# dusanerdeljan/stereo-depth

Hardware: AMD Instinct MI355X
Metric: disparity maps/sec (stereo pairs/sec) at 1242x375 D=128 (higher is better)
Workload: dtype f32

## Files before the change

stereo-depth_amd/csrc/k_match_fast.h:

```cpp
#pragma once
#include "smx_common.h"

namespace smx {

constexpr int FA_HALO = 11;
constexpr int FA_VALID = 64 - 2 * FA_HALO;
#ifndef SMX_FA_WAVES
#define SMX_FA_WAVES 4
#endif
constexpr int FA_WAVES = SMX_FA_WAVES;
#ifndef SMX_FA_DS_WAVES
#define SMX_FA_DS_WAVES 8
#endif
constexpr int FA_DS_WAVES = SMX_FA_DS_WAVES;
#ifndef SMX_FA_TH
#define SMX_FA_TH 24
#endif
constexpr int FA_TH = SMX_FA_TH;
#ifndef SMX_FA_TH_SMALL
#define SMX_FA_TH_SMALL 8
#endif
constexpr int FA_TH_SMALL = SMX_FA_TH_SMALL;
constexpr int FA_TH_SMALL_TALL = 12;
constexpr int FA_TH_SMALL_MID = 10;
#ifndef SMX_FA_PF
#define SMX_FA_PF 2
#endif
constexpr int FA_PF = SMX_FA_PF;
#ifndef SMX_FA_SB_PERIOD
#define SMX_FA_SB_PERIOD 2
#endif
#ifndef SMX_FA_OCC
#define SMX_FA_OCC 3
#endif
#ifndef SMX_FA_DS_OCC
#define SMX_FA_DS_OCC 4
#endif
constexpr int FA_WGCOLS = FA_VALID * FA_WAVES + 2 * FA_HALO;
#ifndef SMX_FA_WIDE_FROM
#define SMX_FA_WIDE_FROM (256 - FA_WGCOLS + 1)
#endif
constexpr int FA_WIDE_FROM = SMX_FA_WIDE_FROM;
constexpr int FA_MID_PITCH = 288;
#ifdef SMX_FA_NO_MID_PITCH
constexpr int FA_MID_UPTO = 0;
#else
constexpr int FA_MID_UPTO = FA_MID_PITCH - FA_WGCOLS + 1;
#endif
constexpr int FA_PL = (FA_VALID * FA_WAVES + 2 * FA_HALO + 7) & ~7;
constexpr int FA_BITWORDS = 64;
__host__ __device__ inline int fast_bitwords(int Dd) {
    return Dd > FA_BITWORDS * 32 ? 2 : ((Dd + 1) & ~1);
}
#define SMX_FOR_EACH_NEEDED(tbl, lo, hi, all_needed, lane, dd, rows, BODY)                                      \
    for (int g_ = (lo); g_ < (hi); g_ += 64) {                                                                  \
        const int idx_ = g_ + (lane);                                                                           \
        unsigned word_ = 0u;                                                                                    \
        if (idx_ < (hi)) word_ = (all_needed) ? ~0u : (tbl)[idx_];                                              \
        unsigned long long m_ = __ballot(word_ != 0u);                                                          \
        while (m_ != 0ull) {                                                                                    \
            const int k_ = __builtin_ctzll(m_);                                                                 \
            m_ &= m_ - 1ull;                                                                                    \
            const int dd = g_ + k_;                                                                             \
            const unsigned rows = (unsigned)__builtin_amdgcn_readlane((int)word_, k_);                          \
            BODY                                                                                                \
        }                                                                                                       \
    }

constexpr int FA_DENSE_MAX_TH = 27;
constexpr int FA_XROW = 64 + 12;
#ifndef SMX_FA_XCH_ROWS
#define SMX_FA_XCH_ROWS 2
#endif
constexpr int FA_XCH_ROWS = SMX_FA_XCH_ROWS;
constexpr int FA_XCH_FLOATS = 2 * FA_XCH_ROWS * FA_XROW;

__host__ __device__ constexpr int fast_merge_rows(int th) { return th > 8 ? (th + 1) / 2 : th; }

template <int PR> inline size_t fast_lds_bytes(int th, int Dd, bool dsplit = false) {
    const size_t nw = dsplit ? FA_DS_WAVES : FA_WAVES;
    return (size_t)(th + 22) * (FA_PL + PR) * sizeof(unsigned short) + nw * fast_bitwords(Dd) * sizeof(unsigned) +
           nw * FA_XCH_FLOATS * sizeof(float) + (dsplit ? nw * fast_merge_rows(th) * 64 * 2 * sizeof(float) : 0);
}

__device__ __forceinline__ float dpp_shr1(float v) {
    return __int_as_float(__builtin_amdgcn_update_dpp(0, __float_as_int(v), 0x138, 0xf, 0xf, true));
}
__device__ __forceinline__ float dpp_shl1(float v) {
    return __int_as_float(__builtin_amdgcn_update_dpp(0, __float_as_int(v), 0x130, 0xf, 0xf, true));
}
__device__ __forceinline__ unsigned dppu_sum3(unsigned v) {
    unsigned t = (unsigned)__builtin_amdgcn_update_dpp(0, (int)v, 0x138, 0xf, 0xf, true) + v;
    asm("" : "+v"(t));
    return t + (unsigned)__builtin_amdgcn_update_dpp(0, (int)v, 0x130, 0xf, 0xf, true);
}

__device__ __forceinline__ void store_u32off(float *base_uniform, unsigned off_elems, float v) {
    *(float *)((char *)base_uniform + (size_t)(off_elems * 4u)) = v;
}

__device__ __forceinline__ void atomic_or_u32off(unsigned *base_uniform, unsigned off_words, unsigned bits) {
    atomicOr((unsigned *)((char *)base_uniform + (size_t)(off_words * 4u)), bits);
}

template <int NK, int NW, bool ROUND = false>
__device__ __forceinline__ void fast_stage(unsigned short *tile, int pitch, const float *img, int h, int w,
                                           int row0, int col0, int rows, int cols, float unit, int wv, int lane) {
    int cidx[NK];
    {
        int c = wrapi(col0 + lane, w);
        const int cstep = 64 % w;
#pragma unroll
        for (int k = 0; k < NK; ++k) {
            cidx[k] = c;
            c += cstep;
            c = c >= w ? c - w : c;
        }
    }
    int ra = wrapi(row0 + wv, h);
    const int rstep = (2 * NW) % h, rhalf = NW % h;
    for (int r = wv; r < rows; r += 2 * NW) {
        const int r2 = r + NW;
        int rb = ra + rhalf;
        rb = rb >= h ? rb - h : rb;
        const float *src = img + (size_t)ra * w;
        const float *src2 = img + (size_t)(r2 < rows ? rb : ra) * w;
        float v[NK], v2[NK];
#pragma unroll
        for (int k = 0; k < NK; ++k) {
            const bool in = lane + 64 * k < cols;
            v[k] = in ? src[cidx[k]] : 0.f;
            v2[k] = in ? src2[cidx[k]] : 0.f;
        }
        unsigned short *dst = tile + r * pitch, *dst2 = tile + r2 * pitch;
#pragma unroll
        for (int k = 0; k < NK; ++k) {
            if (lane + 64 * k < cols) {
                dst[lane + 64 * k] = (unsigned short)(ROUND ? unit * v[k] + 0.5f : unit * v[k]);
                if (r2 < rows) dst2[lane + 64 * k] = (unsigned short)(ROUND ? unit * v2[k] + 0.5f : unit * v2[k]);
            }
        }
        ra += rstep;
        ra = ra >= h ? ra - h : ra;
    }
}

struct FastLane {
    const unsigned short *lptr, *rptr;
    float *xch;
    unsigned c255;
    float inv;
    bool store_ok;
    int rows_ok;
    int colidx;
    size_t row0;
    size_t plane;
    unsigned *cand;
    unsigned cand_off_a, cand_off_b;
    unsigned long long cand_mask_a, cand_mask_b;
    unsigned cand_rstride;
    int x0;
};

typedef float f32x2 __attribute__((ext_vector_type(2)));
typedef __attribute__((address_space(3))) f32x2 fa_lds_f32x2;

__device__ __forceinline__ void argb_update(int kbyte, int &word, float m, float best, int dsel) {
    if (kbyte == 0)
        asm volatile("v_cmp_gt_f32 vcc, %1, %2\n\tv_cndmask_b32_sdwa %0, %0, %3, vcc dst_sel:BYTE_0 dst_unused:UNUSED_PRESERVE src0_sel:BYTE_0 src1_sel:BYTE_0"
                     : "+v"(word) : "v"(m), "v"(best), "v"(dsel) : "vcc");
    else if (kbyte == 1)
        asm volatile("v_cmp_gt_f32 vcc, %1, %2\n\tv_cndmask_b32_sdwa %0, %0, %3, vcc dst_sel:BYTE_1 dst_unused:UNUSED_PRESERVE src0_sel:BYTE_1 src1_sel:BYTE_0"
                     : "+v"(word) : "v"(m), "v"(best), "v"(dsel) : "vcc");
    else if (kbyte == 2)
        asm volatile("v_cmp_gt_f32 vcc, %1, %2\n\tv_cndmask_b32_sdwa %0, %0, %3, vcc dst_sel:BYTE_2 dst_unused:UNUSED_PRESERVE src0_sel:BYTE_2 src1_sel:BYTE_0"
                     : "+v"(word) : "v"(m), "v"(best), "v"(dsel) : "vcc");
    else
        asm volatile("v_cmp_gt_f32 vcc, %1, %2\n\tv_cndmask_b32_sdwa %0, %0, %3, vcc dst_sel:BYTE_3 dst_unused:UNUSED_PRESERVE src0_sel:BYTE_3 src1_sel:BYTE_0"
                     : "+v"(word) : "v"(m), "v"(best), "v"(dsel) : "vcc");
}

template <int TH, int PR, bool P1ONLY, int PK16, int MODE = 0, bool ARGB = false, bool DENSE = false>
__device__ __forceinline__ void fast_pass_pair(const MatchParams &p, const FastLane &ln, int d,
                                               bool valid_b, float (&best)[TH], int (&arg)[TH],
                                               const unsigned short *rptr_b_in = nullptr, int db = 0,
                                               const unsigned *argpk = nullptr, int am_a = 0, int ap_a = 0,
                                               int am_b = 0, int ap_b = 0, const unsigned *vpk = nullptr,
                                               unsigned *hits = nullptr, unsigned rowmask = ~0u,
                                               float *dmb = nullptr, float *dma = nullptr, float *dcp = nullptr,
                                               float *dfirst = nullptr) {
    constexpr int NQ = TH + 20;
    f32x2 s1 = {0.f, 0.f}, s2 = {0.f, 0.f};
    unsigned k1 = 0u, k2 = 0u;
    const unsigned c255pk = ln.c255 * 0x10001u;
    f32x2 r3[NQ], r9[NQ], r21[NQ];
    unsigned lv[TH + 22], rva[TH + 22], rvb[TH + 22];
    f32x2 vs = {0.f, 0.f}, cs = {0.f, 0.f}, hs = {0.f, 0.f};
    f32x2 t_m3 = {0.f, 0.f}, t_p3 = {0.f, 0.f}, u_m6 = {0.f, 0.f}, u_p6 = {0.f, 0.f};
    const int lane_ = threadIdx.x & 63;
#ifdef SMX_FA_ARGMAX2
    int dva = d, dvb = d + 1;
    if (ARGB && MODE == 0) asm volatile("" : "+v"(dva), "+v"(dvb));
#endif
    const unsigned short *rptr_b = (MODE == 0 || MODE == 3) ? ln.rptr - (valid_b ? 1 : 0) : rptr_b_in;
    (void)db;
#pragma unroll
    for (int rr_ = 0; rr_ < TH + 22 + FA_PF; ++rr_) {
        if (rr_ < TH + 22) {
            lv[rr_] = ln.lptr[rr_ * FA_PL];
            rva[rr_] = ln.rptr[rr_ * PR];
            rvb[rr_] = rptr_b[rr_ * PR];
        }
        if (rr_ >= FA_PF) {
            const int r = rr_ - FA_PF;
            f32x2 s0 = {0.f, 0.f};
            unsigned k0 = 0u;
            if (PK16) {
                const unsigned sa = __builtin_amdgcn_sad_u16(lv[r], rva[r], 0u);
                const unsigned sb = __builtin_amdgcn_sad_u16(lv[r], rvb[r], 0u);
                k0 = c255pk - ((sb << 16) | sa);
            } else {
                s0.x = (float)(ln.c255 - __builtin_amdgcn_sad_u16(lv[r], rva[r], 0u));
                s0.y = (float)(ln.c255 - __builtin_amdgcn_sad_u16(lv[r], rvb[r], 0u));
            }
            if (r >= 2) {
                const int q = r - 2;
                f32x2 x3;
                if (PK16 == 2) {
                    const unsigned v3 = (k2 + k1) + k0;
                    const unsigned cv = dppu_sum3(v3);
                    const unsigned y3 = dppu_sum3(cv);
                    x3.x = (float)(y3 & 0xffffu);
                    x3.y = (float)(y3 >> 16);
                } else if (PK16 == 1) {
                    const unsigned v3 = (k2 + k1) + k0;
                    const unsigned cvp = dppu_sum3(v3);
                    f32x2 cv;
                    cv.x = (float)(cvp & 0xffffu);
                    cv.y = (float)(cvp >> 16);
                    x3.x = (dpp_shr1(cv.x) + cv.x) + dpp_shl1(cv.x);
                    x3.y = (dpp_shr1(cv.y) + cv.y) + dpp_shl1(cv.y);
                } else {
                    const f32x2 v3 = (s2 + s1) + s0;
                    f32x2 cv;
                    cv.x = (dpp_shr1(v3.x) + v3.x) + dpp_shl1(v3.x);
                    cv.y = (dpp_shr1(v3.y) + v3.y) + dpp_shl1(v3.y);
                    x3.x = (dpp_shr1(cv.x) + cv.x) + dpp_shl1(cv.x);
                    x3.y = (dpp_shr1(cv.y) + cv.y) + dpp_shl1(cv.y);
                }
                r3[q] = x3;
                if (q >= 12) r9[q - 6] = (t_m3 + r3[q - 6]) + t_p3;
                if (q >= 18) r21[q - 9] = (u_m6 + u_p6) + r3[q - 9];
#ifdef SMX_EXP_NOXCH
                if (q >= 11 && q + 1 < NQ) { t_m3 = r3[q - 5]; t_p3 = r3[q - 4]; }
                if (q >= 17 && q + 1 < NQ) { u_m6 = r9[q - 8]; u_p6 = r9[q - 7]; }
#else
                if (q >= 11 && q + 1 < NQ) {
                    f32x2 *x3b = (f32x2 *)ln.xch + lane_;
                    x3b[6] = r3[q - 5];
                    __builtin_amdgcn_wave_barrier();
                    {
                        const volatile fa_lds_f32x2 *xr = (const volatile fa_lds_f32x2 *)x3b;
                        t_m3 = xr[3]; t_p3 = xr[9];
                    }
                }
                if (q >= 17 && q + 1 < NQ) {
                    f32x2 *x9b = (f32x2 *)(ln.xch + (FA_XCH_ROWS > 1 ? 2 * FA_XROW : 0)) + lane_;
                    x9b[6] = r9[q - 8];
                    __builtin_amdgcn_wave_barrier();
                    {
                        const volatile fa_lds_f32x2 *xr = (const volatile fa_lds_f32x2 *)x9b;
                        u_m6 = xr[0]; u_p6 = xr[12];
                    }
                }
#endif
                vs += r3[q];
                if (q >= 21) vs -= r3[q - 21];
                if (q >= 12) cs += r9[q - 6];
                if (q >= 21) cs -= r9[q - 15];
                if (q >= 18) hs += r21[q - 9];
                if (q >= 21) hs -= r21[q - 12];
                if (q >= 20) {
                    const int o = q - 20;
                    const f32x2 agg = (hs * vs) * cs;
                    if ((MODE == 1 || MODE == 2) && !((rowmask >> o) & 1u)) {
                    } else if (MODE == 2) {
                        unsigned upk_w = argpk[o >> 1], vpk_w = vpk[o >> 1];
                        asm volatile("" : "+v"(upk_w), "+v"(vpk_w));
                        const unsigned U = (upk_w >> (16 * (o & 1))) & 0xffffu;
                        const unsigned V = (vpk_w >> (16 * (o & 1))) & 0xffffu;
                        int ci = ln.colidx;
                        asm volatile("" : "+v"(ci));
                        const unsigned off = (unsigned)(o * p.w + ci);
                        float *cp = p.costs + ln.row0;
                        auto put = [&](unsigned dl1, unsigned o2, float v) {
                            const size_t pl = dl1 == 1u ? 0 : (dl1 == 2u ? 1 : 2);
                            cp[pl * ln.plane + o2] = v * ln.inv;
                        };
                        const unsigned a1 = (unsigned)(d + 1) - U, a2 = V + 1u - (unsigned)d, a3 = (unsigned)(am_a + 1) - U;
                        const unsigned b1 = (unsigned)(db + 1) - U, b2 = V + 1u - (unsigned)db;
                        if (a1 < 3u) put(a1, off, agg.x);
                        if (a2 < 3u) put(a2, off + 1u, agg.x);
                        if (a3 < 3u) put(a3, off, agg.x);
                        if (b1 < 3u) put(b1, off, agg.y);
                        if (b2 < 3u) put(b2, off + 1u, agg.y);
                    } else if (MODE == 4) {
                        best[o] = __builtin_fmaxf(__builtin_fmaxf(best[o], agg.x), agg.y);
                    } else if (MODE == 3) {
                        const bool okp = ln.store_ok && o < ln.rows_ok;
                        const unsigned long long ma = __ballot(okp && agg.x >= best[o]);
                        const unsigned long long mb = __ballot(okp && agg.y >= best[o]);
                        const unsigned tr = (unsigned)(((ln.x0 + o) >> 4) - (ln.x0 >> 4));
                        const unsigned h4 = ((ma & ln.cand_mask_a) != 0ull ? 1u : 0u) | ((ma & ln.cand_mask_b) != 0ull ? 2u : 0u) |
                                            ((mb & ln.cand_mask_a) != 0ull ? 4u : 0u) | ((mb & ln.cand_mask_b) != 0ull ? 8u : 0u);
                        *hits |= h4 << (4u * tr);
                    } else if (MODE == 1) {
                        const int a = (int)((argpk[o >> 1] >> (16 * (o & 1))) & 0xffffu);
                        int ci = ln.colidx;
                        asm volatile("" : "+v"(ci));
                        const unsigned off = (unsigned)(o * p.w + ci);
                        const bool xa = a == am_a, xb = a == ap_a;
                        if (xa || a == am_b) store_u32off(p.costs + ln.row0 + ln.plane, off, (xa ? agg.x : agg.y) * ln.inv);
                        if (xb || a == ap_b) store_u32off(p.costs + ln.row0 + 2 * ln.plane, off, (xb ? agg.x : agg.y) * ln.inv);
                    } else {
                        if constexpr (DENSE) {
                            const float after_d = valid_b ? agg.y : __builtin_nanf("");
                            dma[o] = (dma[o] != dma[o]) ? agg.x : dma[o];
                            const bool ca = (agg.x > best[o]) | (d == 0);
                            const float b1 = __builtin_fmaxf(best[o], agg.x);
                            dmb[o] = ca ? dcp[o] : dmb[o];
                            dma[o] = ca ? after_d : dma[o];
                            const bool cb = agg.y > b1;
                            dmb[o] = cb ? agg.x : dmb[o];
                            dma[o] = cb ? __builtin_nanf("") : dma[o];
                            dcp[o] = agg.y;
                            if (dfirst) dfirst[o] = agg.x;
                        }
#if !defined(SMX_FA_ARGMAX2)
                        const float m = __builtin_fmaxf(__builtin_fmaxf(best[o], agg.x), agg.y);
                        const int dsel = (agg.x == m) ? d : d + 1;
#ifndef SMX_EXP_NOARG
                        if (ARGB) {
                            argb_update(o & 3, arg[o >> 2], m, best[o], dsel);
                        } else {
                            const bool changed = m > best[o];
                            arg[o] = changed ? dsel : arg[o];
                        }
#else
                        (void)dsel;
#endif
                        best[o] = m;
#else
                        if (ARGB) {
                            argb_update(o & 3, arg[o >> 2], agg.x, best[o], dva);
                            best[o] = __builtin_fmaxf(best[o], agg.x);
                            argb_update(o & 3, arg[o >> 2], agg.y, best[o], dvb);
                            best[o] = __builtin_fmaxf(best[o], agg.y);
                        } else {
                            const float m = __builtin_fmaxf(__builtin_fmaxf(best[o], agg.x), agg.y);
                            const int dsel = (agg.x == m) ? d : d + 1;
                            arg[o] = m > best[o] ? dsel : arg[o];
                            best[o] = m;
                        }
#endif
                    }
                }
            }
            s2 = s1;
            s1 = s0;
            k2 = k1;
            k1 = k0;
        }
        if ((rr_ % SMX_FA_SB_PERIOD) == SMX_FA_SB_PERIOD - 1)
            __builtin_amdgcn_sched_barrier(0);
    }
}

constexpr int FA_STAT_WG_STRIDE_DS = 16;
template <bool DSPLIT>
__device__ __forceinline__ void fast_stats_report(const MatchParams &p, int b, int wg_lin, int wv, int marches, bool window) {
    if (!p.fast_stats || b % p.fast_stride != 0) return;
    if (DSPLIT && wg_lin % FA_STAT_WG_STRIDE_DS != 0) return;
    const bool win = window && (!DSPLIT || wv == 0);
    const unsigned long long v = ((unsigned long long)(unsigned)marches << 24) | (win ? 1ull : 0ull);
    if (v != 0ull) (void)__hip_atomic_fetch_add(p.fast_stats, v, __ATOMIC_RELAXED, __HIP_MEMORY_SCOPE_AGENT);
}

template <int TU, int NH, int PR, int PK16, class StageRight>
__device__ __forceinline__ void fast_stacked_tail(const MatchParams &p, const BlockIdx3 &blk, const FastLane &ln, const float (&best)[TU * NH],
                                                  const int (&argb)[TU * NH], const unsigned short *Rt, unsigned *bits, int wcol, int x0,
                                                  bool active, StageRight &&stage_right) {
    constexpr int ND = PR - FA_WGCOLS + 1;
    const int lane = threadIdx.x & 63, wv = threadIdx.x >> 6;
    const int h = p.h, w = p.w, Dd = p.Dd, BW = fast_bitwords(Dd);
    const bool all_needed = Dd > FA_BITWORDS * 32;
    unsigned *wbits = bits + wv * BW;
#pragma unroll
    for (int hh = 0; hh < NH; ++hh) {
        float bh[TU];
        int ah[TU];
#pragma unroll
        for (int o = 0; o < TU; ++o) {
            bh[o] = best[hh * TU + o];
            ah[o] = (argb[(hh * TU + o) >> 2] >> (8 * ((hh * TU + o) & 3))) & 0xff;
        }
        FastLane lh = ln;
        lh.lptr = ln.lptr + hh * TU * FA_PL;
        lh.row0 = ln.row0 + (size_t)(hh * TU) * w;
        lh.rows_ok = max(0, min(TU, h - x0 - hh * TU));
        const unsigned short *Rh = Rt + hh * TU * PR;
        unsigned dup_left = 0u;
#ifndef SMX_FA_NO_DEDUP
        if (!all_needed) {
#pragma unroll
            for (int o = 0; o < TU; ++o) {
                const int la = __builtin_amdgcn_update_dpp(-1, ah[o], 0x138, 0xf, 0xf, false);
                dup_left |= (la == ah[o] ? 1u : 0u) << o;
            }
            const int left_ok = __builtin_amdgcn_update_dpp(0, lh.store_ok ? 1 : 0, 0x138, 0xf, 0xf, false);
            if (!left_ok) dup_left = 0u;
        }
#endif
        if (lh.store_ok) {
#pragma unroll
            for (int o = 0; o < TU; ++o) {
                if (o < lh.rows_ok) {
                    const unsigned off = (unsigned)(o * w + lh.colidx);
                    store_u32off(p.wta + lh.row0, off, (float)ah[o] + (float)p.dmin);
                    const bool nv = !(bh[o] > SMX_FLT_MIN);
                    store_u32off(p.costs + lh.row0, off, nv ? 0.0f : bh[o] * lh.inv);
                    if (!all_needed && !((dup_left >> o) & 1u)) {
                        const int dn = (ah[o] + 1 == Dd) ? 0 : ah[o] + 1;
                        const int dp = (ah[o] == 0) ? Dd - 1 : ah[o] - 1;
                        atomicOr(&wbits[dn], 1u << o);
                        atomicOr(&wbits[dp], 1u << o);
                    }
                }
            }
        }
        int marches2 = 0;
        unsigned argpk[(TU + 1) / 2];
#pragma unroll
        for (int o = 0; o < (TU + 1) / 2; ++o) argpk[o] = 0u;
#pragma unroll
        for (int o = 0; o < TU; ++o)
            argpk[o >> 1] |= ((lh.store_ok && o < lh.rows_ok) ? (unsigned)ah[o] : 0xffffu) << (16 * (o & 1));
        for (int d0 = 0; d0 < Dd; d0 += ND) {
            const int nd = min(ND, Dd - d0);
            if (Dd > ND) stage_right(d0, nd);
            else __syncthreads();
            if (active) {
                auto march = [&](int dda, int ddb, unsigned rows) {
                    const int da = d0 + dda, db = d0 + ddb;
                    ++marches2;
                    lh.rptr = Rh + wcol + lane + (nd - 1 - dda);
                    fast_pass_pair<TU, PR, false, PK16, 1>(p, lh, da, false, bh, ah, Rh + wcol + lane + (nd - 1 - ddb), db, argpk,
                                                           da == 0 ? Dd - 1 : da - 1, da + 1 == Dd ? 0 : da + 1,
                                                           db == 0 ? Dd - 1 : db - 1, db + 1 == Dd ? 0 : db + 1, nullptr, nullptr, rows);
                };
                int pend = -1;
                unsigned pend_rows = 0u;
                SMX_FOR_EACH_NEEDED(wbits + d0, 0, nd, all_needed, lane, dd, rows, {
                    if (pend < 0) { pend = dd; pend_rows = rows; }
                    else { march(pend, dd, pend_rows | rows); pend = -1; }
                })
                if (pend >= 0) march(pend, pend, pend_rows);
            }
        }
        if (lane == 0) fast_stats_report<false>(p, blk.z, (int)(blk.x + gridDim.x * blk.y), wv, marches2, active && lh.rows_ok > 0);
        if (hh + 1 < NH)
            for (int e = lane; e < BW; e += 64) wbits[e] = 0u;
    }
}

template <int TH, int PR, bool P1ONLY, bool DSPLIT, int PK16, bool ARGB = false, bool DENSE = false>
__device__ __forceinline__ void match_fast_body(const MatchParams &p, const BlockIdx3 &blk) {
    static_assert(!DENSE || !P1ONLY, "the dense form is a pass 1 with neighbours: min_disparity = 0");
    static_assert(!DENSE || !DSPLIT || !ARGB, "latency shape: one register per winner");
    constexpr int NW = DSPLIT ? FA_DS_WAVES : FA_WAVES;
    constexpr int WGCOLS = DSPLIT ? 64 : FA_WGCOLS;
    constexpr int ND = PR - WGCOLS + 1;
    constexpr int NH = TH > 32 ? 2 : 1;
    constexpr int TU = TH / NH;
    static_assert(NH == 1 || (TH == 2 * TU && TU <= 32 && ARGB && !DSPLIT && !DENSE && !P1ONLY),
                  "stacked bands: two unit bands, byte-packed winners, throughput shape, sparse form");
    const int b = blk.z;

    extern __shared__ __attribute__((aligned(16))) unsigned short fsmem[];
    unsigned short *Lt = fsmem;
    unsigned short *Rt = fsmem + (TH + 22) * FA_PL;
    unsigned *bits = (unsigned *)(Rt + (TH + 22) * PR);
    const int BW = fast_bitwords(p.Dd);

    const int tid = threadIdx.x;
    const int lane = tid & 63;
    const int wv = tid >> 6;
    const int h = p.h, w = p.w, Dd = p.Dd;
    const int cwg0 = blk.x * (DSPLIT ? 1 : FA_WAVES) * FA_VALID;
    const int cw0 = cwg0 + (DSPLIT ? 0 : wv * FA_VALID);
    const int wcol = DSPLIT ? 0 : wv * FA_VALID;
    const bool active = cw0 < w;
    const int x0 = blk.y * TH;
    const int col = cw0 - FA_HALO + lane;
    const float *Lp = p.Ld + (size_t)b * h * w;
    const float *Rp = p.Rd + (size_t)b * h * w;
    const float unit = p.unit;

    FastLane ln;
    ln.xch = (float *)(bits + NW * BW) + wv * FA_XCH_FLOATS;
    ln.c255 = (unsigned)(255.0f * unit);
    ln.inv = 1.0f / (unit * unit * unit);
    ln.store_ok = active && lane >= FA_HALO && lane < FA_HALO + FA_VALID && col < w;
    ln.rows_ok = min(TH, h - x0);
    ln.plane = (size_t)p.B * h * w;
    ln.row0 = ((size_t)b * h + x0) * w;
    ln.colidx = ln.store_ok ? col : 0;
    ln.lptr = Lt + wcol + lane;

    float best[TH];
    int arg[TH];
#pragma unroll
    for (int o = 0; o < TH; ++o) { best[o] = SMX_FLT_MIN; arg[o] = 0; }
    float dmb[DENSE ? TH : 1], dma[DENSE ? TH : 1], dcp[DENSE ? TH : 1];
    float dfirst[DENSE && DSPLIT ? TH : 1];
#pragma unroll
    for (int o = 0; o < (DENSE ? TH : 1); ++o) { dmb[o] = 0.f; dma[o] = 0.f; dcp[o] = 0.f; }
#pragma unroll
    for (int o = 0; o < (DENSE && DSPLIT ? TH : 1); ++o) dfirst[o] = 0.f;

    fast_stage<(WGCOLS + 63) / 64, NW>(Lt, FA_PL, Lp, h, w, x0 - FA_HALO, cwg0 - FA_HALO, TH + 22, WGCOLS, unit, wv, lane);
    for (int e = tid; e < NW * BW; e += 64 * NW) bits[e] = 0u;

    auto stage_right = [&](int d0, int nd) {
        __syncthreads();
        const int cbase = cwg0 - FA_HALO - (p.dmin + d0 + nd - 1);
        fast_stage<(PR + 63) / 64, NW>(Rt, PR, Rp, h, w, x0 - FA_HALO, cbase, TH + 22, WGCOLS + nd - 1, unit, wv, lane);
        __syncthreads();
    };

    for (int d0 = 0; d0 < Dd; d0 += ND) {
        const int nd = min(ND, Dd - d0);
        stage_right(d0, nd);
        if (active) {
            const int q4 = ((nd + 2 * NW - 1) / (2 * NW)) * 2;
            const int dd_lo = DSPLIT ? min(nd, wv * q4) : 0;
            const int dd_hi = DSPLIT ? min(nd, dd_lo + q4) : nd;
            for (int dd = dd_lo; dd < dd_hi; dd += 2) {
                ln.rptr = Rt + wcol + lane + (nd - 1 - dd);
                if constexpr (DENSE)
                    fast_pass_pair<TH, PR, P1ONLY, PK16, 0, ARGB, true>(p, ln, d0 + dd, dd + 1 < dd_hi, best, arg, nullptr, 0, nullptr,
                                                                         0, 0, 0, 0, nullptr, nullptr, ~0u, dmb, dma, dcp,
                                                                         DSPLIT && dd == dd_lo ? dfirst : nullptr);
                else
                    fast_pass_pair<TH, PR, P1ONLY, PK16, 0, ARGB>(p, ln, d0 + dd, dd + 1 < dd_hi, best, arg);
            }
        }
    }
    if constexpr (NH > 1) {
        fast_stacked_tail<TU, NH, PR, PK16>(p, blk, ln, best, arg, Rt, bits, wcol, x0, active, stage_right);
        return;
    }
    if (ARGB) {
        int packed[(TH + 3) / 4];
#pragma unroll
        for (int o = 0; o < (TH + 3) / 4; ++o) packed[o] = arg[o];
#pragma unroll
        for (int o = 0; o < TH; ++o) arg[o] = (packed[o >> 2] >> (8 * (o & 3))) & 0xff;
    }
    float *mrg = (float *)(bits + NW * BW) + NW * FA_XCH_FLOATS;
    if constexpr (DSPLIT && DENSE) {
        constexpr int MR = fast_merge_rows(TH), R2 = (NW * MR * 2) / (NW * 6);
        static_assert(R2 >= 1 && R2 <= NW, "merge buffer: at least one row of six values per wave");
        const int q4 = ((Dd + 2 * NW - 1) / (2 * NW)) * 2;
        const int nk = (Dd + q4 - 1) / q4;
#pragma unroll 1
        for (int o0 = 0; o0 < TH; o0 += R2) {
            __syncthreads();
#pragma unroll
            for (int o = 0; o < TH; ++o) {
                if (o >= o0 && o < o0 + R2) {
                    float *q = mrg + ((size_t)(wv * R2 + (o - o0)) * 64 + lane) * 6;
                    q[0] = best[o]; q[1] = __int_as_float(arg[o]); q[2] = dmb[o]; q[3] = dma[o]; q[4] = dfirst[o]; q[5] = dcp[o];
                }
            }
            __syncthreads();
            const int j = wv;
            if (j < R2 && o0 + j < ln.rows_ok && ln.store_ok) {
                auto M = [&](int k, int f) { return mrg[((size_t)(k * R2 + j) * 64 + lane) * 6 + f]; };
                float bb = SMX_FLT_MIN;
                int aa = 0, kw = 0;
                for (int k = 0; k < nk; ++k) {
                    const float bk = M(k, 0);
                    const bool g = bk > bb;
                    aa = g ? __float_as_int(M(k, 1)) : aa;
                    kw = g ? k : kw;
                    bb = g ? bk : bb;
                }
                float mb = M(kw, 2), ma = M(kw, 3);
                if (aa == kw * q4) mb = M(kw > 0 ? kw - 1 : nk - 1, 5);
                if (ma != ma) ma = M(kw + 1 < nk ? kw + 1 : 0, 4);
                const unsigned off = (unsigned)((o0 + j) * w + ln.colidx);
                store_u32off(p.wta + ln.row0, off, (float)aa + (float)p.dmin);
                store_u32off(p.costs + ln.row0, off, !(bb > SMX_FLT_MIN) ? 0.0f : bb * ln.inv);
                store_u32off(p.costs + ln.row0 + ln.plane, off, ma * ln.inv);
                store_u32off(p.costs + ln.row0 + 2 * ln.plane, off, mb * ln.inv);
            }
        }
        return;
    }
    if (DSPLIT) {
        constexpr int MR = fast_merge_rows(TH);
#pragma unroll
        for (int o0 = 0; o0 < TH; o0 += MR) {
            __syncthreads();
#pragma unroll
            for (int o = o0; o < o0 + MR && o < TH; ++o) {
                mrg[((wv * MR + (o - o0)) * 64 + lane) * 2] = best[o];
                mrg[((wv * MR + (o - o0)) * 64 + lane) * 2 + 1] = __int_as_float(arg[o]);
            }
            __syncthreads();
#pragma unroll
            for (int o = o0; o < o0 + MR && o < TH; ++o) {
                float bb = SMX_FLT_MIN;
                int aa = 0;
#pragma unroll
                for (int k = 0; k < NW; ++k) {
                    const float bk = mrg[((k * MR + (o - o0)) * 64 + lane) * 2];
                    const int ak = __float_as_int(mrg[((k * MR + (o - o0)) * 64 + lane) * 2 + 1]);
                    const bool g = bk > bb;
                    aa = g ? ak : aa;
                    bb = g ? bk : bb;
                }
                best[o] = bb;
                arg[o] = aa;
            }
        }
    }

    const bool all_needed = Dd > FA_BITWORDS * 32;
    unsigned dup_left = 0u;
#ifndef SMX_FA_NO_DEDUP
    if (!DENSE && !P1ONLY && !all_needed) {
#pragma unroll
        for (int o = 0; o < TH; ++o) {
            const int la = __builtin_amdgcn_update_dpp(-1, arg[o], 0x138, 0xf, 0xf, false);
            dup_left |= (la == arg[o] ? 1u : 0u) << o;
        }
        const int left_ok = __builtin_amdgcn_update_dpp(0, ln.store_ok ? 1 : 0, 0x138, 0xf, 0xf, false);
        if (!left_ok) dup_left = 0u;
    }
#endif
    if (ln.store_ok) {
        unsigned *wbits = bits + (DSPLIT ? 0 : wv) * BW;
#pragma unroll
        for (int o = 0; o < TH; ++o) {
            if (o < ln.rows_ok && (!DSPLIT || o % NW == wv)) {
                const unsigned off = (unsigned)(o * w + ln.colidx);
                store_u32off(p.wta + ln.row0, off, (float)arg[o] + (float)p.dmin);
                const bool nv = !(best[o] > SMX_FLT_MIN);
                store_u32off(p.costs + ln.row0, off, nv ? 0.0f : best[o] * ln.inv);
                if constexpr (DENSE) {
                    store_u32off(p.costs + ln.row0 + 2 * ln.plane, off, (arg[o] == 0 ? dcp[o] : dmb[o]) * ln.inv);
                    if (dma[o] != dma[o]) {
                        if (!all_needed) atomicOr(&wbits[0], 1u << o);
                    } else {
                        store_u32off(p.costs + ln.row0 + ln.plane, off, dma[o] * ln.inv);
                    }
                } else
                if (!P1ONLY && !all_needed && !((dup_left >> o) & 1u)) {
                    const int dn = (arg[o] + 1 == Dd) ? 0 : arg[o] + 1;
                    const int dp = (arg[o] == 0) ? Dd - 1 : arg[o] - 1;
                    atomicOr(&wbits[dn], 1u << o);
                    atomicOr(&wbits[dp], 1u << o);
                }
            }
        }
    }
    if (P1ONLY) return;

    int marches2 = 0;
    unsigned argpk[(TH + 1) / 2];
#pragma unroll
    for (int o = 0; o < (TH + 1) / 2; ++o) argpk[o] = 0u;
#pragma unroll
    for (int o = 0; o < TH; ++o)
        argpk[o >> 1] |= ((ln.store_ok && o < ln.rows_ok) ? (unsigned)arg[o] : 0xffffu) << (16 * (o & 1));
    for (int d0 = 0; d0 < (DENSE ? 1 : Dd); d0 += ND) {
        const int nd = min(ND, Dd - d0);
        if (Dd > ND) stage_right(d0, nd);
        else __syncthreads();
        if (active) {
            const unsigned *mybits = bits + (DSPLIT ? 0 : wv) * BW;
            const int q4 = ((nd + 2 * NW - 1) / (2 * NW)) * 2;
            const int dd_lo = DSPLIT ? min(nd, wv * q4) : 0;
            const int dd_hi = DSPLIT ? min(nd, dd_lo + q4) : nd;
            auto march = [&](int dda, int ddb, unsigned rows) {
                const int da = d0 + dda, db = d0 + ddb;
                ++marches2;
                ln.rptr = Rt + wcol + lane + (nd - 1 - dda);
                fast_pass_pair<TH, PR, false, PK16, 1>(p, ln, da, false, best, arg, Rt + wcol + lane + (nd - 1 - ddb), db, argpk,
                                                       da == 0 ? Dd - 1 : da - 1, da + 1 == Dd ? 0 : da + 1,
                                                       db == 0 ? Dd - 1 : db - 1, db + 1 == Dd ? 0 : db + 1, nullptr, nullptr, rows);
            };
            int pend = -1;
            unsigned pend_rows = 0u;
#ifndef SMX_EXP_NOPASS2
            if constexpr (DSPLIT) {
                (void)dd_lo; (void)dd_hi;
                int seen = 0;
                SMX_FOR_EACH_NEEDED(mybits + d0, 0, nd, all_needed, lane, dd, rows, {
                    const bool mine = (seen >> 1) % NW == wv;
                    ++seen;
                    if (mine) {
                        if (pend < 0) { pend = dd; pend_rows = rows; }
                        else { march(pend, dd, pend_rows | rows); pend = -1; }
                    }
                })
            } else {
                SMX_FOR_EACH_NEEDED(mybits + d0, dd_lo, dd_hi, all_needed, lane, dd, rows, {
                    if (pend < 0) { pend = dd; pend_rows = rows; }
                    else { march(pend, dd, pend_rows | rows); pend = -1; }
                })
            }
#endif
            if (pend >= 0) march(pend, pend, pend_rows);
        }
    }
    if constexpr (!DENSE) {
        if (lane == 0) fast_stats_report<DSPLIT>(p, b, (int)(blk.x + gridDim.x * blk.y), wv, marches2, active);
    }
}

#ifdef SMX_FA_NUM_VGPR
#define SMX_FA_VGPR_ATTR __attribute__((amdgpu_num_vgpr(SMX_FA_NUM_VGPR)))
#else
#define SMX_FA_VGPR_ATTR
#endif
template <int TH, int PR, bool P1ONLY, bool DSPLIT, int PK16, bool ARGB, bool DENSE = false>
__global__ __launch_bounds__(64 * (DSPLIT ? FA_DS_WAVES : FA_WAVES), DENSE ? 2 : (DSPLIT ? (TH >= FA_TH_SMALL_TALL ? 2 : SMX_FA_DS_OCC) : SMX_FA_OCC)) SMX_FA_VGPR_ATTR void k_match_fast(MatchParams p) {
    const BlockIdx3 blk = xcd_block_index();
    if ((p.gate == 1 && p.flags[blk.z] == p.epoch) || (p.gate == 2 && p.flags[blk.z] != p.epoch)) {
        return;
    }
    match_fast_body<TH, PR, P1ONLY, DSPLIT, PK16, ARGB, DENSE>(p, blk);
}

inline int fast_pk(int unit) { return unit <= 4 ? 2 : (unit <= 16 ? 1 : 0); }
inline bool fast_small_wide(int Dd) { return Dd > 256 - 64 + 1; }

template <int TH, int PR, bool P1ONLY, bool DSPLIT, bool ARGB, bool DENSE>
inline void launch_match_fast_k(int pk, dim3 grid, dim3 block, size_t lds, const MatchParams &p, hipStream_t s) {
    if (pk == 2) hipLaunchKernelGGL((k_match_fast<TH, PR, P1ONLY, DSPLIT, 2, ARGB, DENSE>), grid, block, lds, s, p);
    else if (pk == 1) hipLaunchKernelGGL((k_match_fast<TH, PR, P1ONLY, DSPLIT, 1, ARGB, DENSE>), grid, block, lds, s, p);
    else hipLaunchKernelGGL((k_match_fast<TH, PR, P1ONLY, DSPLIT, 0, ARGB, DENSE>), grid, block, lds, s, p);
}

template <int TH, int PR, bool DSPLIT, bool ARGB>
inline void launch_match_fast_a(const FastLaunch &fl, const MatchParams &p, int n, hipStream_t s) {
    const int win_per_wg = DSPLIT ? 1 : FA_WAVES;
    const dim3 grid((p.w + FA_VALID * win_per_wg - 1) / (FA_VALID * win_per_wg), (p.h + TH - 1) / TH, n);
    const size_t lds = fast_lds_bytes<PR>(TH, p.Dd, DSPLIT);
    const dim3 block(64 * (DSPLIT ? FA_DS_WAVES : FA_WAVES));
#ifdef SMX_FA_FORCE_TH
    if (lds > 64 * 1024) {
        (void)hipFuncSetAttribute(reinterpret_cast<const void *>(&k_match_fast<TH, PR, false, DSPLIT, 2, ARGB>),
                                  hipFuncAttributeMaxDynamicSharedMemorySize, (int)lds);
    }
#endif
    if (fl.form == FAST_DENSE_SMALL) {
        if constexpr (DSPLIT && TH == FA_TH_SMALL_TALL) launch_match_fast_k<TH, PR, false, true, false, true>(fl.pk, grid, block, lds, p, s);
    } else if (fl.form == FAST_DENSE) {
        if constexpr (!DSPLIT && ARGB && TH <= FA_DENSE_MAX_TH) launch_match_fast_k<TH, PR, false, false, ARGB, true>(fl.pk, grid, block, lds, p, s);
    } else if (fl.form == FAST_PASS1_ONLY) {
        launch_match_fast_k<TH, PR, true, DSPLIT, ARGB, false>(fl.pk, grid, block, lds, p, s);
    } else {
        launch_match_fast_k<TH, PR, false, DSPLIT, ARGB, false>(fl.pk, grid, block, lds, p, s);
    }
}

template <int TH, int PR, bool DSPLIT>
inline void launch_match_fast_t(const FastLaunch &fl, const MatchParams &p, int n, hipStream_t s) {
    if constexpr (DSPLIT) {
        launch_match_fast_a<TH, PR, true, false>(fl, p, n, s);
    } else if constexpr (PR == 256 || PR == FA_MID_PITCH) {
        launch_match_fast_a<TH, PR, false, true>(fl, p, n, s);
    } else {
        if (fl.argb) launch_match_fast_a<TH, PR, false, true>(fl, p, n, s);
        else launch_match_fast_a<TH, PR, false, false>(fl, p, n, s);
    }
}

__host__ __device__ constexpr int fast_tall_pitch(int Dd) { return Dd <= FA_WIDE_FROM ? 256 : (Dd <= FA_MID_UPTO ? FA_MID_PITCH : 320); }

template <int TH>
inline void launch_match_fast_tall(const FastLaunch &fl, const MatchParams &p, int n, hipStream_t s) {
    if (fl.pitch == 256) launch_match_fast_t<TH, 256, false>(fl, p, n, s);
    else if (fl.pitch == FA_MID_PITCH) launch_match_fast_t<TH, FA_MID_PITCH, false>(fl, p, n, s);
    else launch_match_fast_t<TH, 320, false>(fl, p, n, s);
}

constexpr int FA_STACK = 2;
constexpr int FA_STACK_TH = FA_STACK * FA_TH;
template <int PR> inline bool fast_stack_fits(int Dd) {
    const size_t granule = 1280, lds = fast_lds_bytes<PR>(FA_STACK_TH, Dd);
    return 2 * ((lds + granule - 1) / granule * granule) <= 160 * 1024;
}
inline bool fast_stack_instantiated(int pitch, int Dd) { return pitch == 256 && fast_stack_fits<256>(Dd); }

template <int PR>
inline void launch_match_fast_stacked(const FastLaunch &fl, const MatchParams &p, int n, hipStream_t s) {
    const dim3 grid((p.w + FA_VALID * FA_WAVES - 1) / (FA_VALID * FA_WAVES), (p.h + FA_STACK_TH - 1) / FA_STACK_TH, n);
    const size_t lds = fast_lds_bytes<PR>(FA_STACK_TH, p.Dd);
    const dim3 block(64 * FA_WAVES);
    if (fl.pk == 2) hipLaunchKernelGGL((k_match_fast<FA_STACK_TH, PR, false, false, 2, true, false>), grid, block, lds, s, p);
    else if (fl.pk == 1) hipLaunchKernelGGL((k_match_fast<FA_STACK_TH, PR, false, false, 1, true, false>), grid, block, lds, s, p);
    else hipLaunchKernelGGL((k_match_fast<FA_STACK_TH, PR, false, false, 0, true, false>), grid, block, lds, s, p);
}
template <int PR>
inline hipError_t fast_stacked_raise_lds_caps() {
    const int cap = (int)fast_lds_bytes<PR>(FA_STACK_TH, PR - FA_WGCOLS + 1);
    const void *kernels[3] = {reinterpret_cast<const void *>(&k_match_fast<FA_STACK_TH, PR, false, false, 2, true, false>),
                              reinterpret_cast<const void *>(&k_match_fast<FA_STACK_TH, PR, false, false, 1, true, false>),
                              reinterpret_cast<const void *>(&k_match_fast<FA_STACK_TH, PR, false, false, 0, true, false>)};
    for (const void *k : kernels)
        if (hipError_t e = hipFuncSetAttribute(k, hipFuncAttributeMaxDynamicSharedMemorySize, cap); e != hipSuccess) return e;
    return hipSuccess;
}

struct FastPlan {
    bool small;
    int th;
    bool wide;
    int stack = 1;
};

inline FastPlan match_fast_plan(const MatchParams &p, int n, int cus, int stack_opt = -1) {
    FastPlan pl{};
    const long wgs_tall = (long)((p.w + FA_VALID * FA_WAVES - 1) / (FA_VALID * FA_WAVES)) * ((p.h + FA_TH - 1) / FA_TH) * n;
    pl.small = 8 * wgs_tall < (p.on_lanes ? 8L : 13L) * cus;
    if (pl.small) {
        pl.th = FA_TH_SMALL;
        pl.wide = fast_small_wide(p.Dd);
        const long windows = (long)((p.w + FA_VALID - 1) / FA_VALID) * n;
        const long wg_small = windows * ((p.h + FA_TH_SMALL - 1) / FA_TH_SMALL), wg_tall = windows * ((p.h + FA_TH_SMALL_TALL - 1) / FA_TH_SMALL_TALL);
        if (wg_small > cus && wg_tall <= cus) {
            pl.th = FA_TH_SMALL_TALL;
#ifndef SMX_FA_NO_MID
#ifdef SMX_FA_MID_P1
        } else {
#else
        } else if (!p.pass1_only) {
#endif
            const long wg_mid = windows * ((p.h + FA_TH_SMALL_MID - 1) / FA_TH_SMALL_MID), slots = 2L * cus;
            const long r_small = (wg_small + slots - 1) / slots, r_mid = (wg_mid + slots - 1) / slots;
            if (r_mid * (FA_TH_SMALL_MID + 22) < r_small * (FA_TH_SMALL + 22)) pl.th = FA_TH_SMALL_MID;
#endif
        }
        return pl;
    }
    pl.wide = p.Dd > FA_WIDE_FROM;
    const int cand[3] = {24, 27, 32};
    int best = 24;
    long best_rows = -1;
    for (int th : cand) {
        const int pr = fast_tall_pitch(p.Dd);
        const size_t lds = pr == 256 ? fast_lds_bytes<256>(th, p.Dd) : (pr == FA_MID_PITCH ? fast_lds_bytes<FA_MID_PITCH>(th, p.Dd) : fast_lds_bytes<320>(th, p.Dd));
        const size_t granule = 1280;
        const bool three_per_cu = 3 * ((lds + granule - 1) / granule * granule) <= 160 * 1024;
        const long rows = (long)((p.h + th - 1) / th) * (th + 22) * (th == 32 ? 106 : 100) * (three_per_cu ? 100 : 130);
        if (best_rows < 0 || rows < best_rows) { best_rows = rows; best = th; }
    }
    pl.th = best;
#ifdef SMX_FA_FORCE_TH
    pl.th = SMX_FA_FORCE_TH;
#endif
    if (stack_opt != 0 && !p.dense && !p.pass1_only && fast_stack_instantiated(fast_tall_pitch(p.Dd), p.Dd)) {
        const long rows_stack = (long)((p.h + FA_STACK_TH - 1) / FA_STACK_TH) * (FA_STACK_TH + 22);
        if (stack_opt == 1 || (p.on_lanes && rows_stack < (long)((p.h + pl.th - 1) / pl.th) * (pl.th + 22))) {
            pl.th = FA_TH;
            pl.stack = FA_STACK;
        }
    }
    return pl;
}

}
```

stereo-depth_amd/csrc/k_match_filter.h:

```cpp
#pragma once
#include "k_match_fast.h"

namespace smx {

inline double filter_error_bound_units(double u) {
    const double Hmax = 63.0 * 2295.0, Cmax = 81.0 * 2295.0;
    const double eH = 567.0 / u, eC = 729.0 / u;
    const double rounding = 2.0 * eH * Hmax * Cmax + Hmax * Hmax * eC;
    return (1.05 * rounding + 1e-4 * Hmax * Hmax * Cmax) * u * u * u;
}

#ifndef SMX_FILTER_A_GAP
#define SMX_FILTER_A_GAP 1
#endif
constexpr int FILTER_A_GAP = SMX_FILTER_A_GAP;
constexpr int FILTER_TILE_H = 16, FILTER_TILE_W = 128;
__host__ __device__ inline int filter_cand_words(int Dd) { return (Dd + 31) / 32; }

template <int PR> inline size_t filter_lds_bytes(int th) {
    return (size_t)(th + 22) * (FA_PL + PR) * sizeof(unsigned short) + FA_WAVES * FA_XCH_FLOATS * sizeof(float);
}

struct FilterParams {
    unsigned *cand;
    int tiles_x, tiles_y, cw;
    float two_e;
    const int *range_flags;
};

template <int TH, int PR, int PK16>
__global__ __launch_bounds__(64 * FA_WAVES, SMX_FA_OCC) void k_match_filter(MatchParams p, FilterParams f) {
    const BlockIdx3 blk = xcd_block_index();
    const int b = blk.z;
    if (f.range_flags[b] == p.epoch) return;
    constexpr int NW = FA_WAVES;
    constexpr int WGCOLS = FA_WGCOLS;
    constexpr int ND = PR - WGCOLS + 1;

    extern __shared__ __attribute__((aligned(16))) unsigned short fsmem[];
    unsigned short *Lt = fsmem;
    unsigned short *Rt = fsmem + (TH + 22) * FA_PL;
    float *xch = (float *)(Rt + (TH + 22) * PR);

    const int tid = threadIdx.x, lane = tid & 63, wv = tid >> 6;
    const int h = p.h, w = p.w, Dd = p.Dd;
    const int cwg0 = blk.x * NW * FA_VALID;
    const int cw0 = cwg0 + wv * FA_VALID;
    const int wcol = wv * FA_VALID;
    const bool active = cw0 < w;
    const int x0 = blk.y * TH;
    const int col = cw0 - FA_HALO + lane;
    const float *Lp = p.Ld + (size_t)b * h * w;
    const float *Rp = p.Rd + (size_t)b * h * w;
    const float unit = p.unit;

    FastLane ln;
    ln.xch = xch + wv * FA_XCH_FLOATS;
    ln.c255 = (unsigned)(255.0f * unit);
    ln.inv = 1.0f;
    ln.store_ok = active && lane >= FA_HALO && lane < FA_HALO + FA_VALID && col < w;
    ln.rows_ok = min(TH, h - x0);
    ln.plane = 0;
    ln.row0 = 0;
    ln.colidx = ln.store_ok ? col : 0;
    ln.lptr = Lt + wcol + lane;
    ln.cand = f.cand + (size_t)b * f.tiles_y * f.tiles_x * f.cw;
    {
        const int ta = cw0 / FILTER_TILE_W;
        const unsigned long long valid = __ballot(ln.store_ok);
        const unsigned long long in_a = __ballot(ln.store_ok && col / FILTER_TILE_W == ta);
        ln.cand_mask_a = in_a;
        ln.cand_mask_b = valid & ~in_a;
        ln.cand_off_a = (unsigned)(ta * f.cw);
        ln.cand_off_b = (unsigned)((ta + 1) * f.cw);
    }
    ln.cand_rstride = (unsigned)(f.tiles_x * f.cw);
    ln.x0 = x0;

    float best[TH];
    int arg[TH];
#pragma unroll
    for (int o = 0; o < TH; ++o) { best[o] = SMX_FLT_MIN; arg[o] = 0; }

    fast_stage<(WGCOLS + 63) / 64, NW, true>(Lt, FA_PL, Lp, h, w, x0 - FA_HALO, cwg0 - FA_HALO, TH + 22, WGCOLS, unit, wv, lane);
    auto stage_right = [&](int d0, int nd) {
        __syncthreads();
        const int cbase = cwg0 - FA_HALO - (p.dmin + d0 + nd - 1);
        fast_stage<(PR + 63) / 64, NW, true>(Rt, PR, Rp, h, w, x0 - FA_HALO, cbase, TH + 22, WGCOLS + nd - 1, unit, wv, lane);
        __syncthreads();
    };

    for (int d0 = 0; d0 < Dd; d0 += ND) {
        const int nd = min(ND, Dd - d0);
        stage_right(d0, nd);
        if (active) {
            for (int dd = 0; dd < nd; dd += 2 * FILTER_A_GAP) {
                const int ddb = dd + FILTER_A_GAP < nd ? dd + FILTER_A_GAP : dd;
                ln.rptr = Rt + wcol + lane + (nd - 1 - dd);
                fast_pass_pair<TH, PR, true, PK16, 4>(p, ln, d0 + dd, ddb != dd, best, arg, Rt + wcol + lane + (nd - 1 - ddb));
            }
        }
    }
#pragma unroll
    for (int o = 0; o < TH; ++o) best[o] = best[o] - f.two_e;

    for (int d0 = 0; d0 < Dd; d0 += ND) {
        const int nd = min(ND, Dd - d0);
        if (Dd > ND) stage_right(d0, nd);
        if (active) {
            for (int dd = 0; dd < nd; dd += 2) {
                const bool vb = dd + 1 < nd;
                ln.rptr = Rt + wcol + lane + (nd - 1 - dd);
                const int da = d0 + dd, db = vb ? da + 1 : da;
                unsigned hits = 0u;
                fast_pass_pair<TH, PR, true, PK16, 3>(p, ln, da, vb, best, arg, nullptr, db, nullptr, 0, 0, 0, 0, nullptr, &hits);
                hits = __builtin_amdgcn_readfirstlane(hits);
                if (hits != 0u && lane == FA_HALO) {
                    for (unsigned tr = 0; tr < 3; ++tr) {
                        const unsigned h4 = (hits >> (4u * tr)) & 15u;
                        const unsigned rowoff = ((unsigned)(x0 >> 4) + tr) * ln.cand_rstride;
                        if (h4 & 1u) atomic_or_u32off(ln.cand, ln.cand_off_a + rowoff + ((unsigned)da >> 5), 1u << (da & 31));
                        if (h4 & 2u) atomic_or_u32off(ln.cand, ln.cand_off_b + rowoff + ((unsigned)da >> 5), 1u << (da & 31));
                        if (h4 & 4u) atomic_or_u32off(ln.cand, ln.cand_off_a + rowoff + ((unsigned)db >> 5), 1u << (db & 31));
                        if (h4 & 8u) atomic_or_u32off(ln.cand, ln.cand_off_b + rowoff + ((unsigned)db >> 5), 1u << (db & 31));
                    }
                }
            }
        }
    }
}


template <int TH, int PR>
inline void launch_match_filter_t(int pk, const MatchParams &p, const FilterParams &f, int n, hipStream_t s) {
    const dim3 grid((p.w + FA_VALID * FA_WAVES - 1) / (FA_VALID * FA_WAVES), (p.h + TH - 1) / TH, n), block(64 * FA_WAVES);
    const size_t lds = filter_lds_bytes<PR>(TH);
    if (pk == 2) hipLaunchKernelGGL((k_match_filter<TH, PR, 2>), grid, block, lds, s, p, f);
    else if (pk == 1) hipLaunchKernelGGL((k_match_filter<TH, PR, 1>), grid, block, lds, s, p, f);
    else hipLaunchKernelGGL((k_match_filter<TH, PR, 0>), grid, block, lds, s, p, f);
}

struct FilterPlan { int th; bool wide; };
inline FilterPlan filter_plan(const MatchParams &p, int n, int cus) {
    const long colwgs = (p.w + FA_VALID * FA_WAVES - 1) / (FA_VALID * FA_WAVES);
    FilterPlan best{27, false};
    double best_cost = -1.0;
    for (int wide = 0; wide < 2; ++wide) {
        const int nd = (wide ? 320 : 256) - FA_WGCOLS + 1;
        const int chunks = (p.Dd + nd - 1) / nd;
        for (int th : {24, 27, 32}) {
            const size_t lds = wide ? filter_lds_bytes<320>(th) : filter_lds_bytes<256>(th);
            const bool three = 3 * ((lds + 1279) / 1280 * 1280) <= 160 * 1024;
            const double r = (double)(colwgs * ((p.h + th - 1) / th) * n) / (three ? 3.0 * cus : 2.0 * cus);
            const double rounds = r <= 2.0 ? (double)(long)(r + 0.999999) : r;
            const double cost = rounds * (th + 22) * (three ? 1.0 : 0.87) * (1.0 + 0.03 * (chunks - 1));
            if (best_cost < 0.0 || cost < best_cost) { best_cost = cost; best = FilterPlan{th, wide != 0}; }
        }
    }
    return best;
}

}
```

Before: 99700.

## Use exact float prefix sums for vertical box-filter windows in match pass

```diff
diff --git a/stereo-depth_amd/csrc/k_match_fast.h b/stereo-depth_amd/csrc/k_match_fast.h
--- a/stereo-depth_amd/csrc/k_match_fast.h
+++ b/stereo-depth_amd/csrc/k_match_fast.h
@@ -76,6 +76,20 @@
 constexpr int FA_XCH_FLOATS = 2 * FA_XCH_ROWS * FA_XROW;
 
 __host__ __device__ constexpr int fast_merge_rows(int th) { return th > 8 ? (th + 1) / 2 : th; }
+
+__host__ __device__ constexpr bool fast_prefix_exact(int th, int k_max) {
+    return (long long)(th + 11) * 48195 * k_max * k_max < (1LL << 24);
+}
+__host__ __device__ constexpr bool fast_prefix_form(int th, int pr, bool p1only, bool dsplit, int pk16, bool argb, bool dense) {
+#ifdef SMX_FA_NO_PREFIX
+    return false;
+#else
+    if (pk16 != 2 || !fast_prefix_exact(th, 2)) return false;
+    if (dsplit) return th == FA_TH_SMALL_TALL;
+    (void)pr; (void)p1only; (void)argb; (void)dense;
+    return true;
+#endif
+}
 
 template <int PR> inline size_t fast_lds_bytes(int th, int Dd, bool dsplit = false) {
     const size_t nw = dsplit ? FA_DS_WAVES : FA_WAVES;
@@ -180,7 +194,7 @@
                      : "+v"(word) : "v"(m), "v"(best), "v"(dsel) : "vcc");
 }
 
-template <int TH, int PR, bool P1ONLY, int PK16, int MODE = 0, bool ARGB = false, bool DENSE = false>
+template <int TH, int PR, bool P1ONLY, int PK16, int MODE = 0, bool ARGB = false, bool DENSE = false, bool PREFIX = false>
 __device__ __forceinline__ void fast_pass_pair(const MatchParams &p, const FastLane &ln, int d,
                                                bool valid_b, float (&best)[TH], int (&arg)[TH],
                                                const unsigned short *rptr_b_in = nullptr, int db = 0,
@@ -189,7 +203,9 @@
                                                unsigned *hits = nullptr, unsigned rowmask = ~0u,
                                                float *dmb = nullptr, float *dma = nullptr, float *dcp = nullptr,
                                                float *dfirst = nullptr) {
+    static_assert(!PREFIX || (PK16 == 2 && fast_prefix_exact(TH, 2)), "prefix form: K <= 2 and every prefix below 2^24");
     constexpr int NQ = TH + 20;
+    constexpr int Q9 = PREFIX ? 11 : 12, Q21 = PREFIX ? 17 : 18;
     f32x2 s1 = {0.f, 0.f}, s2 = {0.f, 0.f};
     unsigned k1 = 0u, k2 = 0u;
     const unsigned c255pk = ln.c255 * 0x10001u;
@@ -248,14 +264,15 @@
                     x3.x = (dpp_shr1(cv.x) + cv.x) + dpp_shl1(cv.x);
                     x3.y = (dpp_shr1(cv.y) + cv.y) + dpp_shl1(cv.y);
                 }
-                r3[q] = x3;
-                if (q >= 12) r9[q - 6] = (t_m3 + r3[q - 6]) + t_p3;
-                if (q >= 18) r21[q - 9] = (u_m6 + u_p6) + r3[q - 9];
+                if (PREFIX && q > 0) r3[q] = r3[q > 0 ? q - 1 : 0] + x3;
+                else r3[q] = x3;
+                if (q >= Q9) r9[q - 6] = (t_m3 + r3[q - 6]) + t_p3;
+                if (q >= Q21) r21[q - 9] = (u_m6 + u_p6) + r3[q - 9];
 #ifdef SMX_EXP_NOXCH
-                if (q >= 11 && q + 1 < NQ) { t_m3 = r3[q - 5]; t_p3 = r3[q - 4]; }
-                if (q >= 17 && q + 1 < NQ) { u_m6 = r9[q - 8]; u_p6 = r9[q - 7]; }
+                if (q >= Q9 - 1 && q + 1 < NQ) { t_m3 = r3[q - 5]; t_p3 = r3[q - 4]; }
+                if (q >= Q21 - 1 && q + 1 < NQ) { u_m6 = r9[q - 8]; u_p6 = r9[q - 7]; }
 #else
-                if (q >= 11 && q + 1 < NQ) {
+                if (q >= Q9 - 1 && q + 1 < NQ) {
                     f32x2 *x3b = (f32x2 *)ln.xch + lane_;
                     x3b[6] = r3[q - 5];
                     __builtin_amdgcn_wave_barrier();
@@ -264,7 +281,7 @@
                         t_m3 = xr[3]; t_p3 = xr[9];
                     }
                 }
-                if (q >= 17 && q + 1 < NQ) {
+                if (q >= Q21 - 1 && q + 1 < NQ) {
                     f32x2 *x9b = (f32x2 *)(ln.xch + (FA_XCH_ROWS > 1 ? 2 * FA_XROW : 0)) + lane_;
                     x9b[6] = r9[q - 8];
                     __builtin_amdgcn_wave_barrier();
@@ -274,12 +291,20 @@
                     }
                 }
 #endif
-                vs += r3[q];
-                if (q >= 21) vs -= r3[q - 21];
-                if (q >= 12) cs += r9[q - 6];
-                if (q >= 21) cs -= r9[q - 15];
-                if (q >= 18) hs += r21[q - 9];
-                if (q >= 21) hs -= r21[q - 12];
+                if (PREFIX) {
+                    if (q >= 20) {
+                        vs = q >= 21 ? r3[q] - r3[q - 21] : r3[q];
+                        cs = r9[q - 6] - r9[q - 15];
+                        hs = r21[q - 9] - r21[q - 12];
+                    }
+                } else {
+                    vs += r3[q];
+                    if (q >= 21) vs -= r3[q - 21];
+                    if (q >= 12) cs += r9[q - 6];
+                    if (q >= 21) cs -= r9[q - 15];
+                    if (q >= 18) hs += r21[q - 9];
+                    if (q >= 21) hs -= r21[q - 12];
+                }
                 if (q >= 20) {
                     const int o = q - 20;
                     const f32x2 agg = (hs * vs) * cs;
@@ -386,7 +411,7 @@
     if (v != 0ull) (void)__hip_atomic_fetch_add(p.fast_stats, v, __ATOMIC_RELAXED, __HIP_MEMORY_SCOPE_AGENT);
 }
 
-template <int TU, int NH, int PR, int PK16, class StageRight>
+template <int TU, int NH, int PR, int PK16, bool PREFIX, class StageRight>
 __device__ __forceinline__ void fast_stacked_tail(const MatchParams &p, const BlockIdx3 &blk, const FastLane &ln, const float (&best)[TU * NH],
                                                   const int (&argb)[TU * NH], const unsigned short *Rt, unsigned *bits, int wcol, int x0,
                                                   bool active, StageRight &&stage_right) {
@@ -454,7 +479,7 @@
                     const int da = d0 + dda, db = d0 + ddb;
                     ++marches2;
                     lh.rptr = Rh + wcol + lane + (nd - 1 - dda);
-                    fast_pass_pair<TU, PR, false, PK16, 1>(p, lh, da, false, bh, ah, Rh + wcol + lane + (nd - 1 - ddb), db, argpk,
+                    fast_pass_pair<TU, PR, false, PK16, 1, false, false, PREFIX>(p, lh, da, false, bh, ah, Rh + wcol + lane + (nd - 1 - ddb), db, argpk,
                                                            da == 0 ? Dd - 1 : da - 1, da + 1 == Dd ? 0 : da + 1,
                                                            db == 0 ? Dd - 1 : db - 1, db + 1 == Dd ? 0 : db + 1, nullptr, nullptr, rows);
                 };
@@ -482,6 +507,7 @@
     constexpr int ND = PR - WGCOLS + 1;
     constexpr int NH = TH > 32 ? 2 : 1;
     constexpr int TU = TH / NH;
+    constexpr bool PREFIX = fast_prefix_form(TH, PR, P1ONLY, DSPLIT, PK16, ARGB, DENSE);
     static_assert(NH == 1 || (TH == 2 * TU && TU <= 32 && ARGB && !DSPLIT && !DENSE && !P1ONLY),
                   "stacked bands: two unit bands, byte-packed winners, throughput shape, sparse form");
     const int b = blk.z;
@@ -548,16 +574,16 @@
             for (int dd = dd_lo; dd < dd_hi; dd += 2) {
                 ln.rptr = Rt + wcol + lane + (nd - 1 - dd);
                 if constexpr (DENSE)
-                    fast_pass_pair<TH, PR, P1ONLY, PK16, 0, ARGB, true>(p, ln, d0 + dd, dd + 1 < dd_hi, best, arg, nullptr, 0, nullptr,
+                    fast_pass_pair<TH, PR, P1ONLY, PK16, 0, ARGB, true, PREFIX>(p, ln, d0 + dd, dd + 1 < dd_hi, best, arg, nullptr, 0, nullptr,
                                                                          0, 0, 0, 0, nullptr, nullptr, ~0u, dmb, dma, dcp,
                                                                          DSPLIT && dd == dd_lo ? dfirst : nullptr);
                 else
-                    fast_pass_pair<TH, PR, P1ONLY, PK16, 0, ARGB>(p, ln, d0 + dd, dd + 1 < dd_hi, best, arg);
+                    fast_pass_pair<TH, PR, P1ONLY, PK16, 0, ARGB, false, PREFIX>(p, ln, d0 + dd, dd + 1 < dd_hi, best, arg);
             }
         }
     }
     if constexpr (NH > 1) {
-        fast_stacked_tail<TU, NH, PR, PK16>(p, blk, ln, best, arg, Rt, bits, wcol, x0, active, stage_right);
+        fast_stacked_tail<TU, NH, PR, PK16, PREFIX>(p, blk, ln, best, arg, Rt, bits, wcol, x0, active, stage_right);
         return;
     }
     if (ARGB) {
@@ -698,7 +724,7 @@
                 const int da = d0 + dda, db = d0 + ddb;
                 ++marches2;
                 ln.rptr = Rt + wcol + lane + (nd - 1 - dda);
-                fast_pass_pair<TH, PR, false, PK16, 1>(p, ln, da, false, best, arg, Rt + wcol + lane + (nd - 1 - ddb), db, argpk,
+                fast_pass_pair<TH, PR, false, PK16, 1, false, false, PREFIX>(p, ln, da, false, best, arg, Rt + wcol + lane + (nd - 1 - ddb), db, argpk,
                                                        da == 0 ? Dd - 1 : da - 1, da + 1 == Dd ? 0 : da + 1,
                                                        db == 0 ? Dd - 1 : db - 1, db + 1 == Dd ? 0 : db + 1, nullptr, nullptr, rows);
             };
diff --git a/stereo-depth_amd/csrc/k_match_filter.h b/stereo-depth_amd/csrc/k_match_filter.h
--- a/stereo-depth_amd/csrc/k_match_filter.h
+++ b/stereo-depth_amd/csrc/k_match_filter.h
@@ -36,6 +36,7 @@
     constexpr int NW = FA_WAVES;
     constexpr int WGCOLS = FA_WGCOLS;
     constexpr int ND = PR - WGCOLS + 1;
+    constexpr bool PREFIX = fast_prefix_form(TH, PR, true, false, PK16, false, false);
 
     extern __shared__ __attribute__((aligned(16))) unsigned short fsmem[];
     unsigned short *Lt = fsmem;
@@ -97,7 +98,7 @@
             for (int dd = 0; dd < nd; dd += 2 * FILTER_A_GAP) {
                 const int ddb = dd + FILTER_A_GAP < nd ? dd + FILTER_A_GAP : dd;
                 ln.rptr = Rt + wcol + lane + (nd - 1 - dd);
-                fast_pass_pair<TH, PR, true, PK16, 4>(p, ln, d0 + dd, ddb != dd, best, arg, Rt + wcol + lane + (nd - 1 - ddb));
+                fast_pass_pair<TH, PR, true, PK16, 4, false, false, PREFIX>(p, ln, d0 + dd, ddb != dd, best, arg, Rt + wcol + lane + (nd - 1 - ddb));
             }
         }
     }
@@ -113,7 +114,7 @@
                 ln.rptr = Rt + wcol + lane + (nd - 1 - dd);
                 const int da = d0 + dd, db = vb ? da + 1 : da;
                 unsigned hits = 0u;
-                fast_pass_pair<TH, PR, true, PK16, 3>(p, ln, da, vb, best, arg, nullptr, db, nullptr, 0, 0, 0, 0, nullptr, &hits);
+                fast_pass_pair<TH, PR, true, PK16, 3, false, false, PREFIX>(p, ln, da, vb, best, arg, nullptr, db, nullptr, 0, 0, 0, 0, nullptr, &hits);
                 hits = __builtin_amdgcn_readfirstlane(hits);
                 if (hits != 0u && lane == FA_HALO) {
                     for (unsigned tr = 0; tr < 3; ++tr) {
```

Measured after the change: 102,300 (median of 6 runs). 2.7% higher.
